# cure-lab/MagicDrive

Measured on AMD Instinct MI355X. Metric: 6-view scenes/sec at 224x400, 50-step DDIM, higher is better.
Workload: dtype bf16; 1 GPU; configs[1]: 6-view 224x400, text-only conditioning (camera_param=None -> CFG off), 50-step DDIM, bf16; scenes_per_gpu=64, ddim_steps=50, scheduler=ddim, parallelism=scene-sharded x1, hipgraph=True, streams=2, output_type=latent

## Files before the change

### include/mdx.h

```cpp
#ifndef MDX_H_
#define MDX_H_

#include <stdint.h>

#ifdef __cplusplus
extern "C" {
#endif

#define MDX_OK 0
#define MDX_EINVAL (-1)
#define MDX_ELAUNCH (-2)
#define MDX_EUNSUPPORTED (-3)

#define MDX_ABI_VERSION 12

#define MDX_EPI_NONE 0
#define MDX_EPI_GEGLU 1
#define MDX_EPI_SILU 2

typedef struct MdxGemmDesc {
    const void* A; const void* W; void* C; const void* R;
    const float* bias; const float* temb; const int32_t* sel_ptr; float* ws;
    int64_t M, N, K;
    int64_t lda, ldw, ldc, ldr;
// ... 32 lines not shown
    const void* X; const void* Wt; void* Y; const void* R;
    const float* bias; const float* temb; const int32_t* sel_ptr; void* reserved_p;
    int64_t B, Hi, Wi, Cin, Ho, Wo, Cout;
    int64_t kh, kw, sh, sw, ph, pw;
    int64_t ldx, ldy, ldr;
    int64_t temb_sel_stride, temb_b_stride;
    int64_t epilogue, x_is_f32, y_is_f32, reserved0;
} MdxConvDirectDesc;
int mdx_conv2d_direct(const MdxConvDirectDesc* d, void* stream);

typedef struct MdxAttnDesc {
    const void* Q; const void* K; const void* Vt; void* O;
    const int32_t* kvmap; const int32_t* tk_dev;
    int64_t B, H, Tq, Tk, d, nsrc;
    int64_t ldq, sQ, ldk, sK, ldv, sV, ldo, sO;
    double scale;
    int64_t joint;
    int64_t q_prescaled;
    int64_t causal;
    int64_t v_rowmajor;
} MdxAttnDesc;
int mdx_attention_bf16(const MdxAttnDesc* d, void* stream);
int mdx_attention_ctx_rows_bf16(const MdxAttnDesc* d, void* stream);

typedef struct MdxGroupNormDesc {
    const void* X; void* Y; const float* gamma; const float* beta;
    int64_t B, HW, C, G, ldx, ldy;
    double eps;
    int64_t silu;
    float* ws; int64_t ws_bytes;
} MdxGroupNormDesc;
int mdx_groupnorm_bf16(const MdxGroupNormDesc* d, void* stream);

typedef struct MdxLayerNormDesc {
    const void* X; void* Y; const float* gamma; const float* beta;
    int64_t M, C, ldx, ldy;
    double eps;
    int64_t reserved0;
} MdxLayerNormDesc;
int mdx_layernorm_bf16(const MdxLayerNormDesc* d, void* stream);

typedef struct MdxSoftmaxDesc {
    const float* X; void* Y;
    int64_t rows, T, ldx, ldy;
    double scale;
    int64_t reserved0;
} MdxSoftmaxDesc;
int mdx_softmax_rows(const MdxSoftmaxDesc* d, void* stream);

#define MDX_EW_ADD 1
#define MDX_EW_COPY 2
#define MDX_EW_UPSAMPLE 3
#define MDX_EW_NCHW_TO_NHWC 4
#define MDX_EW_NHWC_TO_NCHW 5
#define MDX_EW_SILU 6
#define MDX_EW_SCALE 7
typedef struct MdxEwDesc {
    const void* X; void* Y; const int32_t* ymap; const int32_t* xmap;
    int64_t kind, M, C, ldx, ldy;
    int64_t B, Hi, Wi, Ho, Wo;
    int64_t x_is_f32, y_is_f32;
    double alpha;
} MdxEwDesc;
int mdx_elementwise(const MdxEwDesc* d, void* stream);

typedef struct MdxFourierDesc {
// ... 19 lines not shown
    float* x; const float* eps; const float* coef; int32_t* step_ptr; void* x_in; void* reserved_p;
    int64_t n, cfg;
    double guidance;
    int64_t xin_c, xin_ld;
    const float* gv_cond; const float* gv_noise; const uint8_t* gv_mask;
    int64_t gv_mode, gv_view_elems, gv_last_step;
} MdxDdimDesc;
int mdx_cfg_ddim_step(const MdxDdimDesc* d, void* stream);

typedef struct MdxUniPCDesc {
    float* x; const float* eps; const float* coef; int32_t* step_ptr; void* x_in; float* x_last; float* m1; float* m2;
    int64_t n, cfg;
    double guidance;
    int64_t xin_c, xin_ld;
    const float* gv_cond; const float* gv_noise; const uint8_t* gv_mask;
    int64_t gv_mode, gv_view_elems, gv_last_step;
} MdxUniPCDesc;
int mdx_cfg_unipc_step(const MdxUniPCDesc* d, void* stream);

#define MDX_OP_GEMM 1
#define MDX_OP_CONV 2
#define MDX_OP_CONV_DIRECT 3
#define MDX_OP_ATTN 4
#define MDX_OP_GROUPNORM 5
#define MDX_OP_LAYERNORM 6
#define MDX_OP_EW 7
#define MDX_OP_FOURIER 8
#define MDX_OP_GATHER 9
#define MDX_OP_TIMEEMB 10
#define MDX_OP_DDIM 11
#define MDX_OP_UNIPC 12
#define MDX_OP_SOFTMAX 13
#define MDX_OP_ATTN_ROWS 14

#define MDX_DTYPE_BF16 0
#define MDX_DTYPE_F16 1

#define MDX_OP_BYTES 512
typedef struct MdxOp {
    int64_t opcode;
    int64_t dtype;
    unsigned char desc[MDX_OP_BYTES - 16];
} MdxOp;

int mdx_gemm_f16(const MdxGemmDesc* d, void* stream);
int mdx_conv2d_f16(const MdxConvDesc* d, void* stream);
int mdx_conv2d_direct_f16(const MdxConvDirectDesc* d, void* stream);
int mdx_attention_f16(const MdxAttnDesc* d, void* stream);
int mdx_groupnorm_f16(const MdxGroupNormDesc* d, void* stream);
int mdx_layernorm_f16(const MdxLayerNormDesc* d, void* stream);
int mdx_elementwise_f16(const MdxEwDesc* d, void* stream);
int mdx_fourier_embed_f16(const MdxFourierDesc* d, void* stream);
int mdx_gather_rows_f16(const MdxGatherDesc* d, void* stream);
int mdx_timestep_embedding_f16(const MdxTimeEmbDesc* d, void* stream);
int mdx_cfg_ddim_step_f16(const MdxDdimDesc* d, void* stream);
int mdx_cfg_unipc_step_f16(const MdxUniPCDesc* d, void* stream);
int mdx_softmax_rows_f16(const MdxSoftmaxDesc* d, void* stream);
int mdx_attention_ctx_rows_f16(const MdxAttnDesc* d, void* stream);

int mdx_program_run(const MdxOp* ops, int64_t n, void* stream);

int mdx_graph_create(const MdxOp* ops, int64_t n, void** graph_out);
int mdx_graph_launch(void* graph, void* stream);
int mdx_graph_destroy(void* graph);

int mdx_abi_version(void);
const char* mdx_build_id(void);
const char* mdx_last_error(void);
const char* mdx_last_kernel(void);
int mdx_set_option(const char* key, int64_t value);
int mdx_get_option(const char* key, int64_t* value_out);
const char* mdx_option_name(int64_t index);

int mdx_device_info(int64_t* out3);

#ifdef __cplusplus
}
#endif
#endif
```

### magicdrive_amd/_lib.py

```python
from __future__ import annotations

import ctypes as C
import os
from typing import Dict, List, Tuple

_HERE = os.path.dirname(os.path.abspath(__file__))
LIB_PATH = os.environ.get("MDX_LIB_PATH") or os.path.join(_HERE, "libmdx.so")

ABI_VERSION = 12

OP_GEMM, OP_CONV, OP_CONV_DIRECT, OP_ATTN, OP_GROUPNORM, OP_LAYERNORM = 1, 2, 3, 4, 5, 6
OP_EW, OP_FOURIER, OP_GATHER, OP_TIMEEMB, OP_DDIM, OP_UNIPC, OP_SOFTMAX = 7, 8, 9, 10, 11, 12, 13
OP_ATTN_ROWS = 14
OP_BYTES = 512

EPI_NONE, EPI_GEGLU, EPI_SILU = 0, 1, 2
EW_ADD, EW_COPY, EW_UPSAMPLE, EW_NCHW_TO_NHWC, EW_NHWC_TO_NCHW, EW_SILU, EW_SCALE = 1, 2, 3, 4, 5, 6, 7

P, I, D = C.c_void_p, C.c_int64, C.c_double


def _struct(name: str, fields: List[Tuple[str, object]]):
    return type(name, (C.Structure,), {"_fields_": fields})


def _f(kind, names: str):
    return [(n, kind) for n in names.split()]


MdxGemmDesc = _struct("MdxGemmDesc", _f(P, "A W C R bias temb sel_ptr ws") + _f(I, "M N K lda ldw ldc ldr batch sA sW sC sR "
                      "temb_sel_stride temb_b_stride rows_per_b epilogue splitk c_is_f32 ws_bytes") + _f(P, "Vt") + _f(I, "vt_from vt_T vt_ld vt_stride")
                      + _f(D, "ln_eps") + _f(P, "ln_csum ln_scratch") + _f(P, "rowstat_out") + _f(I, "rowstat_parts") + _f(P, "ln_stats") + _f(I, "ln_stats_parts") + _f(P, "Wq"))
MdxConvDesc = _struct("MdxConvDesc", _f(P, "X Wt Y R bias temb sel_ptr ws") + _f(I, "B Hi Wi Cin Ho Wo Cout kh kw sh sw ph pw "
                      "ldx ldy ldr temb_sel_stride temb_b_stride epilogue splitk ws_bytes upsample2x"))
MdxConvDirectDesc = _struct("MdxConvDirectDesc", _f(P, "X Wt Y R bias temb sel_ptr reserved_p") + _f(I, "B Hi Wi Cin Ho Wo Cout kh kw sh sw ph pw "
                            "ldx ldy ldr temb_sel_stride temb_b_stride epilogue x_is_f32 y_is_f32 reserved0"))
MdxAttnDesc = _struct("MdxAttnDesc", _f(P, "Q K Vt O kvmap tk_dev") + _f(I, "B H Tq Tk d nsrc ldq sQ ldk sK ldv sV ldo sO")
                      + _f(D, "scale") + _f(I, "joint q_prescaled causal v_rowmajor"))
MdxGroupNormDesc = _struct("MdxGroupNormDesc", _f(P, "X Y gamma beta") + _f(I, "B HW C G ldx ldy") + _f(D, "eps") + _f(I, "silu") + _f(P, "ws") + _f(I, "ws_bytes"))
MdxLayerNormDesc = _struct("MdxLayerNormDesc", _f(P, "X Y gamma beta") + _f(I, "M C ldx ldy") + _f(D, "eps") + _f(I, "reserved0"))
MdxEwDesc = _struct("MdxEwDesc", _f(P, "X Y ymap xmap") + _f(I, "kind M C ldx ldy B Hi Wi Ho Wo x_is_f32 y_is_f32") + _f(D, "alpha"))
MdxFourierDesc = _struct("MdxFourierDesc", _f(P, "X Y mask null_feat") + _f(I, "n P F ldy"))
MdxGatherDesc = _struct("MdxGatherDesc", _f(P, "T Y idx mask null_row add") + _f(I, "n C ldt ldy n_rows add_period"))
MdxTimeEmbDesc = _struct("MdxTimeEmbDesc", _f(P, "t Y") + _f(I, "n dim flip_sin_to_cos ldy") + _f(D, "freq_shift max_period"))
MdxDdimDesc = _struct("MdxDdimDesc", _f(P, "x eps coef step_ptr x_in reserved_p") + _f(I, "n cfg") + _f(D, "guidance") + _f(I, "xin_c xin_ld")
                      + _f(P, "gv_cond gv_noise gv_mask") + _f(I, "gv_mode gv_view_elems gv_last_step"))
MdxUniPCDesc = _struct("MdxUniPCDesc", _f(P, "x eps coef step_ptr x_in x_last m1 m2") + _f(I, "n cfg") + _f(D, "guidance") + _f(I, "xin_c xin_ld")
                       + _f(P, "gv_cond gv_noise gv_mask") + _f(I, "gv_mode gv_view_elems gv_last_step"))

MdxSoftmaxDesc = _struct("MdxSoftmaxDesc", _f(P, "X Y") + _f(I, "rows T ldx ldy") + _f(D, "scale") + _f(I, "reserved0"))
DESC_OF_OP = {
    OP_GEMM: MdxGemmDesc, OP_CONV: MdxConvDesc, OP_CONV_DIRECT: MdxConvDirectDesc, OP_ATTN: MdxAttnDesc,
    OP_GROUPNORM: MdxGroupNormDesc, OP_LAYERNORM: MdxLayerNormDesc, OP_EW: MdxEwDesc, OP_FOURIER: MdxFourierDesc,
    OP_GATHER: MdxGatherDesc, OP_TIMEEMB: MdxTimeEmbDesc, OP_DDIM: MdxDdimDesc, OP_UNIPC: MdxUniPCDesc, OP_SOFTMAX: MdxSoftmaxDesc,
}
DTYPE_BF16, DTYPE_F16 = 0, 1
ENTRY_OF_OP = {
    OP_GEMM: "mdx_gemm_bf16", OP_CONV: "mdx_conv2d_bf16", OP_CONV_DIRECT: "mdx_conv2d_direct", OP_ATTN: "mdx_attention_bf16",
    OP_GROUPNORM: "mdx_groupnorm_bf16", OP_LAYERNORM: "mdx_layernorm_bf16", OP_EW: "mdx_elementwise",
    OP_FOURIER: "mdx_fourier_embed", OP_GATHER: "mdx_gather_rows", OP_TIMEEMB: "mdx_timestep_embedding", OP_DDIM: "mdx_cfg_ddim_step",
    OP_UNIPC: "mdx_cfg_unipc_step", OP_SOFTMAX: "mdx_softmax_rows",
    OP_ATTN_ROWS: "mdx_attention_ctx_rows_bf16",
}
def entry_name(opcode: int, dtype: int = DTYPE_BF16) -> str:
    n = ENTRY_OF_OP[opcode]
    if dtype == DTYPE_BF16:
        return n
    return (n[:-5] if n.endswith("_bf16") else n) + "_f16"


EXPORTS = sorted(set(ENTRY_OF_OP.values()) | {entry_name(o, DTYPE_F16) for o in ENTRY_OF_OP} | {
    "mdx_program_run", "mdx_graph_create", "mdx_graph_launch", "mdx_graph_destroy",
    "mdx_abi_version", "mdx_build_id", "mdx_last_error", "mdx_last_kernel", "mdx_device_info", "mdx_set_option", "mdx_get_option", "mdx_option_name"})


class MdxOp(C.Structure):
    _fields_ = [("opcode", I), ("dtype", I), ("desc", C.c_ubyte * (OP_BYTES - 16))]


assert C.sizeof(MdxOp) == OP_BYTES
for _d in DESC_OF_OP.values():
    assert C.sizeof(_d) <= OP_BYTES - 16 and C.sizeof(_d) % 8 == 0


class MdxError(RuntimeError):
    pass


_LIB = None


def lib() -> C.CDLL:
    global _LIB
    if _LIB is not None:
        return _LIB
# ... 132 lines not shown
```

### magicdrive_amd/csrc/api.hip

```cpp
#include <cstring>
#include <mutex>
#include <set>
#include <utility>
#include "launch.h"
#include "options.h"
#include <atomic>
#include <cstdlib>

namespace mdx_rt {
char* error_buffer() {
    static thread_local char buf[512] = {0};
    return buf;
}
char* kernel_tag_buffer() {
    static thread_local char buf[128] = {0};
    return buf;
}
int ensure_dyn_smem(const void* kernel, size_t bytes, const char* what) {
    static std::mutex mu;
    static std::set<std::pair<const void*, int>> done;
    int dev = 0;
    hipError_t e = hipGetDevice(&dev);
    if (e != hipSuccess) return mdx::set_error(MDX_ELAUNCH, "hipGetDevice: %s", hipGetErrorString(e));
    std::lock_guard<std::mutex> lk(mu);
// ... 34 lines not shown
    return -1;
}
}
}
namespace mdx_rt {
int64_t opt(int id) { return mdx::g_opt[id].load(std::memory_order_relaxed); }
}

using namespace mdx;

extern "C" int mdx_set_option(const char* key, int64_t value) {
    const int i = find_opt(key);
    if (i < 0) return set_error(MDX_EINVAL, "mdx_set_option: unknown key '%s' (see magicdrive_amd/csrc/options.h)", key ? key : "(null)");
    g_opt[i].store(value, std::memory_order_relaxed);
    return MDX_OK;
}
extern "C" int mdx_get_option(const char* key, int64_t* value_out) {
    const int i = find_opt(key);
    if (i < 0 || !value_out) return set_error(MDX_EINVAL, "mdx_get_option: unknown key '%s'", key ? key : "(null)");
    *value_out = opt(i);
    return MDX_OK;
}
extern "C" const char* mdx_option_name(int64_t index) { return (index >= 0 && index < OPT_COUNT) ? kOptRows[index].key : nullptr; }

static int run_op(const MdxOp* op, hipStream_t st) {
    const void* d = op->desc;
    if (op->dtype == MDX_DTYPE_F16) {
        switch (op->opcode) {
            case MDX_OP_GEMM: return mdx_gemm_f16((const MdxGemmDesc*)d, st);
            case MDX_OP_CONV: return mdx_conv2d_f16((const MdxConvDesc*)d, st);
            case MDX_OP_CONV_DIRECT: return mdx_conv2d_direct_f16((const MdxConvDirectDesc*)d, st);
            case MDX_OP_ATTN: return mdx_attention_f16((const MdxAttnDesc*)d, st);
            case MDX_OP_GROUPNORM: return mdx_groupnorm_f16((const MdxGroupNormDesc*)d, st);
            case MDX_OP_LAYERNORM: return mdx_layernorm_f16((const MdxLayerNormDesc*)d, st);
            case MDX_OP_EW: return mdx_elementwise_f16((const MdxEwDesc*)d, st);
            case MDX_OP_FOURIER: return mdx_fourier_embed_f16((const MdxFourierDesc*)d, st);
            case MDX_OP_GATHER: return mdx_gather_rows_f16((const MdxGatherDesc*)d, st);
            case MDX_OP_TIMEEMB: return mdx_timestep_embedding_f16((const MdxTimeEmbDesc*)d, st);
            case MDX_OP_DDIM: return mdx_cfg_ddim_step_f16((const MdxDdimDesc*)d, st);
            case MDX_OP_UNIPC: return mdx_cfg_unipc_step_f16((const MdxUniPCDesc*)d, st);
            case MDX_OP_SOFTMAX: return mdx_softmax_rows_f16((const MdxSoftmaxDesc*)d, st);
            case MDX_OP_ATTN_ROWS: return mdx_attention_ctx_rows_f16((const MdxAttnDesc*)d, st);
            default: return set_error(MDX_EINVAL, "unknown opcode %ld", (long)op->opcode);
        }
    }
    if (op->dtype != MDX_DTYPE_BF16) return set_error(MDX_EINVAL, "MdxOp.dtype %ld: 0 (bf16) or 1 (fp16)", (long)op->dtype);
    switch (op->opcode) {
        case MDX_OP_GEMM: return mdx_gemm_bf16((const MdxGemmDesc*)d, st);
        case MDX_OP_CONV: return mdx_conv2d_bf16((const MdxConvDesc*)d, st);
        case MDX_OP_CONV_DIRECT: return mdx_conv2d_direct((const MdxConvDirectDesc*)d, st);
        case MDX_OP_ATTN: return mdx_attention_bf16((const MdxAttnDesc*)d, st);
        case MDX_OP_GROUPNORM: return mdx_groupnorm_bf16((const MdxGroupNormDesc*)d, st);
        case MDX_OP_LAYERNORM: return mdx_layernorm_bf16((const MdxLayerNormDesc*)d, st);
        case MDX_OP_EW: return mdx_elementwise((const MdxEwDesc*)d, st);
        case MDX_OP_FOURIER: return mdx_fourier_embed((const MdxFourierDesc*)d, st);
        case MDX_OP_GATHER: return mdx_gather_rows((const MdxGatherDesc*)d, st);
        case MDX_OP_TIMEEMB: return mdx_timestep_embedding((const MdxTimeEmbDesc*)d, st);
        case MDX_OP_DDIM: return mdx_cfg_ddim_step((const MdxDdimDesc*)d, st);
        case MDX_OP_UNIPC: return mdx_cfg_unipc_step((const MdxUniPCDesc*)d, st);
        case MDX_OP_SOFTMAX: return mdx_softmax_rows((const MdxSoftmaxDesc*)d, st);
        case MDX_OP_ATTN_ROWS: return mdx_attention_ctx_rows_bf16((const MdxAttnDesc*)d, st);
        default: return set_error(MDX_EINVAL, "unknown opcode %ld", (long)op->opcode);
    }
}

extern "C" int mdx_program_run(const MdxOp* ops, int64_t n, void* stream) {
    if (!ops && n > 0) return set_error(MDX_EINVAL, "mdx_program_run: null program");
    for (int64_t i = 0; i < n; ++i) {
        int rc = run_op(&ops[i], (hipStream_t)stream);
        if (rc != MDX_OK) {
            char tmp[400];
            strncpy(tmp, error_buffer(), sizeof(tmp) - 1);
            tmp[sizeof(tmp) - 1] = 0;
            return set_error(rc, "op %ld (opcode %ld): %s", (long)i, (long)ops[i].opcode, tmp);
        }
    }
    return MDX_OK;
}

struct GraphHandle {
    hipGraph_t graph;
    hipGraphExec_t exec;
};

extern "C" int mdx_graph_create(const MdxOp* ops, int64_t n, void** graph_out) {
// ... 60 lines not shown
```

### magicdrive_amd/csrc/launch.h

```cpp
#pragma once
#include <hip/hip_runtime.h>
#include <cstdarg>
#include <cstdio>
#include "../../include/mdx.h"

#if defined(MDX_F16) && MDX_F16
#define mdx_gemm_bf16 mdx_gemm_f16
#define mdx_conv2d_bf16 mdx_conv2d_f16
#define mdx_conv2d_direct mdx_conv2d_direct_f16
#define mdx_attention_bf16 mdx_attention_f16
#define mdx_groupnorm_bf16 mdx_groupnorm_f16
#define mdx_layernorm_bf16 mdx_layernorm_f16
#define mdx_elementwise mdx_elementwise_f16
#define mdx_fourier_embed mdx_fourier_embed_f16
#define mdx_gather_rows mdx_gather_rows_f16
#define mdx_timestep_embedding mdx_timestep_embedding_f16
#define mdx_cfg_ddim_step mdx_cfg_ddim_step_f16
#define mdx_cfg_unipc_step mdx_cfg_unipc_step_f16
#define mdx_softmax_rows mdx_softmax_rows_f16
#endif
#ifdef MDX_ATTN_LONG_ENTRY
#undef mdx_attention_bf16
#if defined(MDX_F16) && MDX_F16
#define mdx_attention_bf16 mdx_attention_long_f16
#else
#define mdx_attention_bf16 mdx_attention_long_bf16
#endif
#endif

namespace mdx_rt {
char* error_buffer();
char* kernel_tag_buffer();
int ensure_dyn_smem(const void* kernel, size_t bytes, const char* what);
}

namespace mdx {

using mdx_rt::error_buffer;
using mdx_rt::kernel_tag_buffer;

inline int set_error(int code, const char* fmt, ...) {
    va_list ap;
    va_start(ap, fmt);
    vsnprintf(error_buffer(), 512, fmt, ap);
// ... 29 lines not shown
```

### magicdrive_amd/csrc/norm.hip

```cpp
#include "common.h"
#include "launch.h"
#include "options.h"

namespace mdx {

struct GNParams {
    const bf16_t* X; bf16_t* Y; const float* gamma; const float* beta;
    int B, HW, C, G; long ldx, ldy; float eps; int silu;
};

constexpr int GN_THREADS = 1024;
constexpr int GN_MAX_CPG = 2560;

__device__ __forceinline__ void block_sum2(float& a, float& b, float* red) {
    a = wave_sum(a);
    b = wave_sum(b);
    const int lane = threadIdx.x & 63, wave = threadIdx.x >> 6;
    __syncthreads();
    if (lane == 0) { red[wave] = a; red[16 + wave] = b; }
    __syncthreads();
    float ta = 0.f, tb = 0.f;
#pragma unroll
    for (int i = 0; i < GN_THREADS / 64; ++i) { ta += red[i]; tb += red[16 + i]; }
    a = ta; b = tb;
// ... 511 lines not shown
            for (int e = 0; e < 8; ++e) { const float x = bf2f(f.h[e]); s1 += x; s2 = __builtin_fmaf(x, x, s2); }
        }
    } else {
        for (int c = lane; c < C; c += 64) { const float x = bf2f(xr[c]); s1 += x; s2 = __builtin_fmaf(x, x, s2); }
    }
    s1 = wave_sum(s1); s2 = wave_sum(s2);
    if (lane == 0) {
        *(float2*)(stat + (long)row * 2) = make_float2(s1, s2);
        for (int k = 1; k < parts; ++k) *(float2*)(stat + ((long)k * M + row) * 2) = make_float2(0.f, 0.f);
    }
}
int launch_rowstat(const bf16_t* X, int M, int C, long ldx, float* stat, int parts, hipStream_t st) {
    if (M <= 0) return MDX_OK;
    hipLaunchKernelGGL(rowstat_kernel, dim3((unsigned)((M + 3) / 4)), dim3(256), 0, st, X, M, C, ldx, stat, parts);
    return check_launch("rowstat_kernel");
}
}

extern "C" int mdx_layernorm_bf16(const MdxLayerNormDesc* d, void* stream) {
    if (!d || !d->X || !d->Y || !d->gamma || !d->beta) return set_error(MDX_EINVAL, "mdx_layernorm_bf16: null operand");
    const char* op = "mdx_layernorm_bf16";
    MDX_NEED(need_multiple(op, "C", d->C, 8)); MDX_NEED(need_multiple(op, "ldx", d->ldx, 8)); MDX_NEED(need_multiple(op, "ldy", d->ldy, 8));
    MDX_NEED(need_aligned(op, "X", d->X, 16)); MDX_NEED(need_aligned(op, "Y", d->Y, 16));
    MDX_NEED(need_aligned(op, "gamma", d->gamma, 16)); MDX_NEED(need_aligned(op, "beta", d->beta, 16));
    MDX_NEED(need_int(op, "M", d->M));
    if (d->C <= 0 || d->ldx < d->C || d->ldy < d->C) return set_error(MDX_EINVAL, "%s: need 0 < C <= ldx, ldy", op);
    if (d->C > 8 * 64 * 4) return set_error(MDX_EUNSUPPORTED, "layernorm: C=%ld > 2048", (long)d->C);
    if (d->M <= 0) return MDX_OK;
    LNParams p;
    p.X = (const bf16_t*)d->X; p.Y = (bf16_t*)d->Y; p.gamma = d->gamma; p.beta = d->beta;
    p.M = (int)d->M; p.C = (int)d->C; p.ldx = d->ldx; p.ldy = d->ldy; p.eps = (float)d->eps;
    return launch_layernorm<true>(p, (hipStream_t)stream);
}
```

### magicdrive_amd/csrc/options.h

```cpp
#pragma once
#include <cstdint>

namespace mdx_rt {
int64_t opt(int id);
}

namespace mdx {

#define MDX_OPTIONS(X) \
    X(ATTN_SWZ, 2, "XCD-aware block order of attention.hip: 0 off, 1 per (view, head), 2 per view (all heads of a view on one XCD)") \
    X(ATTN_NW4_BLOCKS, 256L, "attention.hip: 4-wave workgroups from this many blocks") \
    X(ATTN_NW8_BLOCKS, (1L << 40), "attention.hip: 8-wave workgroups from this many blocks") \
    X(ATTN_NW, 0, "force the waves per workgroup of attention.hip (0 = heuristic)") \
    X(ATTN2, 1, "attention2.hip for head dim 40") \
    X(ATTN3, 0, "only in `make ATTN3=1` builds: tools/attn3/attention3.hip (permute-free P, QK of the next kv tile beside this tile's softmax) for the head-dim-40 FOLD launches: self, cross-view, joint") \
    X(ATTN3_WGS, 0, "attention3.hip: persistent workgroups per XCD (0 = automatic: two per CU)") \
    X(ATTN2_PF, 1, "attention2.hip, head dim 40 FOLD 32-query form: permute-free P (PV on 32x32x16 MFMAs, K rows permuted so that a lane's scores are its PV operand)") \
    X(ATTN2_D80, 2, "attention2.hip for head dim 80: 0 never, 1 always, 2 only the two-source cross-view form") \
    X(ATTN2_FOLD, 1, "attention2.hip: subtract the running maximum inside the QK MFMA when Q is pre-scaled (head dim 40)") \
    X(ATTN2_RES, 1, "attention2.hip: kv sequences of <= 3 tiles (text context) resident in LDS, one workgroup per (view, head) walks the query blocks: 0 off, 1 for launches of >= 1024 (view, head) pairs, 2 whenever supported") \
    X(ATTN2_VIEWMAP, 1, "attention2.hip block order: 1 = all heads and query blocks of a view on one XCD (a row's 128-byte lines are shared by the heads), 0 = per (view, head)") \
    X(ATTN2_QT, 0, "32-query tiles per wave in attention2.hip: 0 = automatic (2; 1 for one-source FOLD launches), 1 / 2 = force") \
    X(CONV_OUT_WS, 1, "direct conv with Cout <= 4 and a long K (conv_out): weight-stationary K-parallel kernel (weights in registers, 16 pixels per wave)") \
    X(GEMM_SWZ, 1, "XCD-aware tile order of the generic kernel") \
    X(GEMM_SMALL_TILES, 1, "generic tile choice for small grids (1-4 scenes per call): 64 x 64 for plain GEMMs up to 1408 such tiles and for convs up to 40 k (tile, slab) units, 128 x 128 for larger convs with M < 2048, 128-row GEGLU from M = 512; 0 = the rounds 1-5 rule (128 rows from M = 2048, else 64 x 128)") \
    X(GEMM_BM, 0, "force the generic tile's rows (64 / 128; 0 = heuristic)") \
    X(GEMM_BN, 0, "force the generic tile's columns (64 / 128; 0 = heuristic)") \
    X(GEMM_PIPE, 1, "software-pipelined fragment reads in the generic 128x128x64 tile") \
    X(EPI_WIDE, 1, "16-byte epilogue accesses when alignment allows") \
    X(GEMM_WS, 1, "gemm_ws.hip: 0 off, 1 when M >= 8192, 2 whenever supported") \
    X(GEMM_XL, 1, "gemm_xl.hip: 0 off, 1 cost model, 2 whenever supported") \
    X(XL_K320, 0, "let XL take the K = 320 projections from gemm_ws.hip") \
    X(XL_MIN_TILES, 64, "fewest 256-row tiles an XL launch must have (round 6: 64; 160 until then — 2...8 scenes per call are 2-6 % faster with the lower bound, 12+ scenes and 1 scene do not care: profiles/r06_lat1_small_grids.log)") \
    X(XL_BN, 0, "force an XL tile width (160 / 256 / 320; 0 = cost model)") \
    X(XL_GEGLU320, 0, "K = 320 GEGLU on the 256-wide XL tile instead of gemm_ws.hip") \
    X(GEMM_BM256, 0, "generic 256x128 8-wave tile from M >= value (0 = never)") \
    X(GEMM_TIMING, 0, "s_memtime stamps of the generic kernel into the op workspace") \
    X(GEMM_BK, 64, "generic tile slab depth (64 or 32)") \
    X(GEMM_FLATTEN, 1, "batched shared-A GEMM as ONE col_split XL launch") \
    X(CONV_CIMAJOR, 1, "channel-block-major K order of implicit-GEMM convs") \
    X(WS_SLOTS, 512, "workgroup slots the gemm_ws M walkers are sized for") \
    X(XL_TIMING, 0, "per-workgroup s_memtime stamps into the op workspace") \
    X(GN_REVERSE, 1, "two-stage GroupNorm: statistics pass reads the tensor back to front (Infinity-Cache reuse between producer / passes)") \
    X(GN_FINALIZE_CHUNKS, 16, "two-stage GroupNorm: with more chunks per image than this the chunk partials are combined once by gn_finalize_kernel (0 = always in the apply pass)") \
    X(GN_ONE_KERNEL_ELEMS, (4L << 20), "GroupNorm tensors of at most this many elements (all images) take the one-launch kernel (one workgroup per (image, group)) instead of the two streaming passes") \
    X(GN_TWO_STAGE, 1, "streaming two-stage GroupNorm for maps >= 32768 elements") \
    X(XL_PERSIST, 1, "256x256 XL GEMMs (plain / GEGLU, optional residual) on the persistent kernel gemm_xlp_kernel") \
    X(XD, 0, "W-direct persistent GEMM (gemm_xd.hip: weights global -> registers, finished tile stored under the next tile's main loop) for the 256x256 XL GEMMs whose descriptor carries Wq (K % 128 == 0, K >= 640); bit-identical to gemm_xlp_kernel, measured 0.89-1.04x of it (profiles/r06_xd_ab.log): off by default") \
    X(XL_RASTER, 2, "XL tile order: 0 row-major, 1 XCD-strided M-tiles, 2 XCD-blocked (M-group x N-group panels per XCD)") \
    X(XL_GM, 0, "XL_RASTER 2: force the M-tiles per panel (0 = cost model, xl_layout.h: raster_shape)") \
    X(XL_GN, 0, "XL_RASTER 2: force the N-tiles per panel (0 = cost model)") \
    X(STREAMS, 2, "host side (pipeline): HIP streams a pipe() call spreads its scene chunks over (chunks of >= 16 scenes, one plan + hipGraph each)") \
    X(PLAN_CACHE, 6, "host side (pipeline): sampler plans (captured graphs + buffers) kept per pipeline (LRU); a multi-stream call pins one plan per chunk") \
    X(CHECK_TIMESTEPS, 0, "host side (schedulers): 1 = a device-resident timestep that is not in the scheduler's list raises (one sync per step) instead of poisoning the sample with NaN") \
    X(LN_FUSE, 1, "MdxGemmDesc.ln_eps: 1 = gemm_ws.hip normalises the rows in-kernel, 0 = always normalise into ln_scratch first (A/B)") \
    X(LN_STATS, 1, "MdxGemmDesc.rowstat_out / ln_stats: 1 = row statistics travel from the producer's store phase to the fused LayerNorm, 0 = round-5 behaviour (nothing emitted, in-kernel sums, GEGLU through ln_scratch) (A/B)")

enum Opt : int {
#define MDX_OPT_ENUM(key, dflt, doc) OPT_##key,
    MDX_OPTIONS(MDX_OPT_ENUM)
#undef MDX_OPT_ENUM
    OPT_COUNT
};

using mdx_rt::opt;

}
```

### magicdrive_amd/engine.py

```python
from __future__ import annotations

from typing import Dict, List, Optional, Sequence, Tuple

import torch

from . import _lib as L
from . import ops as O
from . import packing as PK
from .networks.spec import heads_at

BF16, F32 = torch.bfloat16, torch.float32


def q_prescale(head_dim: int) -> float:
    return float(head_dim) ** -0.5 * 1.4426950408889634


class PackedNet:

    def __init__(self, sd: Dict[str, torch.Tensor], device, dtype=BF16):
        assert dtype in (torch.bfloat16, torch.float16), "the kernels take bf16 or fp16 operands (fp32 accumulate)"
        self.sd = sd
        self.device = device
        self.dtype = dtype
        self.cache: Dict[Tuple, torch.Tensor] = {}

    def has(self, key: str) -> bool:
        return key in self.sd

    def _get(self, tag, keys, fn):
        ck = (tag,) + tuple(keys)
        if ck not in self.cache:
            self.cache[ck] = fn(*[self.sd[k].detach().float() for k in keys]).to(self.device)
        return self.cache[ck]

    def lin(self, key, scale: float = 1.0):
        return self._get(("lin", scale), [key], lambda w: (w.reshape(w.shape[0], -1) * scale).contiguous().to(self.dtype))

    def conv(self, key):
# ... 170 lines not shown
class ActSlice:

    __slots__ = ("parent", "c0", "B", "H", "W", "C")

    def __init__(self, parent: Act, c0: int, c1: int):
        self.parent, self.c0, self.B, self.H, self.W, self.C = parent, c0, parent.B, parent.H, parent.W, c1 - c0

    @property
    def tok(self):
        return self.parent.tok[:, self.c0:self.c0 + self.C]

    @property
    def bhwc(self):
        return self.parent.bhwc[..., self.c0:self.c0 + self.C]

    @property
    def btc(self):
        return self.parent.btc[..., self.c0:self.c0 + self.C]


def upsample_conv_folds(device, fold, Hi: int, Wi: int, Ho: int, Wo: int, cin: int, B: int = 0, ldx: int = 0) -> bool:
    if fold is None:
        fold = torch.device(device).type == "cuda"
    if not (bool(fold) and cin % 64 == 0 and Hi * Wi + 256 < (1 << 24) and PK.upsample_fold_ok(Hi, Ho) and PK.upsample_fold_ok(Wi, Wo)):
        return False
    if B and (Ho != 2 * Hi or Wo != 2 * Wi) and (B * Hi * Wi + Wi + 2) * (ldx or cin) * 2 >= 0x7fff0000:
        return False
    return True


class Builder:

    fold_upsample = None

    def __init__(self, cfg, device, n_views: int, n_cam: int, ws_mb: int = 64, dtype=BF16):
        self.cfg = cfg
        self.device = device
        self.B = n_views
        self.n_cam = n_cam
        self.dtype = dtype
        self.pool = Pool(device, dtype)
        self.ops: List[object] = []
        self.ctx_tk_dev: Optional[torch.Tensor] = None
        self.ctx_tk_per_view = False
        self.ws = torch.empty(ws_mb * 1024 * 1024 // 4, dtype=F32, device=device)
        self.groups = cfg["norm_num_groups"]
        self.eps = cfg["norm_eps"]
        pair = cfg["neighboring_view_pair"]
        pair = {int(k): [int(x) for x in v] for k, v in pair.items()}
        self.nattn = cfg.get("neighboring_attn_type", "add")
        if self.nattn not in ("add", "concat", "self"):
            raise NotImplementedError(f"Unknown type: {self.nattn}")
        counts = [len(pair[c]) for c in range(n_cam)]
        self.xv_counts: Optional[List[int]] = None
        self.xv_bo_scale = 1.0
        if self.nattn == "add":
            for c, n in enumerate(counts):
                if n > 2:
                    raise NotImplementedError(f"neighboring_attn_type 'add': view {c} lists {n} neighbours; the summed cross-view form handles at most 2 per view")
            if max(counts) == 0:
                raise RuntimeError("neighboring_view_pair lists no neighbour for any view: there is no cross-view attention to run (torch.cat(): expected a non-empty list of Tensors)")
            self.xv_nsrc = 1 if all(n == 1 for n in counts) else 2
            if len(set(counts)) == 1:
                self.xv_bo_scale = float(counts[0])
            else:
                self.xv_counts = [counts[i % n_cam] for i in range(n_views)]
        elif self.nattn == "concat":
            if len(set(counts)) != 1 or counts[0] == 0:
                raise RuntimeError(f"neighboring_attn_type 'concat' needs the same, non-zero number of neighbours for every view (got {counts}): "
                                   "the reference's torch.cat of the per-view kv sequences fails too (blocks.py:125-132)")
            self.xv_nsrc = counts[0]
        else:
            self.xv_nsrc = n_cam
        assert self.xv_nsrc <= 8, "joint cross-view attention handles <= 8 sources"
        kv = []
        for i in range(n_views):
            base = (i // n_cam) * n_cam
            srcs = list(range(n_cam)) if self.nattn == "self" else pair[i % n_cam]
            kv += [base + nb for nb in srcs] + [-1] * (self.xv_nsrc - len(srcs))
        self.kvmap = torch.tensor(kv, dtype=torch.int32, device=device)
        self.kvmap._mdx_present = sum(1 for x in kv if x >= 0)

    def emit(self, op):
        self.ops.append(op)
        return op

    def new(self, B, H, W, C) -> Act:
        return Act(self.pool.get((B * H * W, C)), B, H, W, C)

    def free(self, a):
        if isinstance(a, ActSlice):
            return
        self.pool.put(a.t if isinstance(a, Act) else a)

    def groupnorm(self, net, pre, x: Act, eps, silu, name) -> Act:
        y = self.new(x.B, x.H, x.W, x.C)
        self.emit(O.GroupNorm(x.btc, y.btc, net.vec(pre + "weight"), net.vec(pre + "bias"), self.groups, eps, silu, ws=self.ws, name=name))
        return y

    def layernorm(self, net, pre, x: torch.Tensor, name) -> torch.Tensor:
        y = self.pool.get(tuple(x.shape))
        self.emit(O.LayerNorm(x, y, net.vec(pre + "weight"), net.vec(pre + "bias"), 1e-5, name=name))
        return y

    @staticmethod
    def wq_of(W: torch.Tensor, M: int, epilogue: int) -> Optional[torch.Tensor]:
        if W.dim() != 2 or not W.is_contiguous() or epilogue not in (L.EPI_NONE, L.EPI_GEGLU) or not L.get_option("XD"):
            return None
        N, K = W.shape
        if K % 128 or K < 640 or N % 16 or ((M + 255) // 256) * ((N + 255) // 256) < 512:
            return None
        wq = getattr(W, "_mdx_wq", None)
        if wq is None:
            wq = PK.pack_wq(W)
            W._mdx_wq = wq
        return wq

    def gemm(self, A, W, N_out, bias=None, R=None, epilogue=L.EPI_NONE, name="", out=None, **kw) -> torch.Tensor:
        C = out if out is not None else self.pool.get((A.shape[0], N_out))
        if "Wq" not in kw and not any(kw.get(k) is not None for k in ("Vt", "temb", "rowstat")) and not kw.get("ln_eps"):
            kw["Wq"] = self.wq_of(W, A.shape[0], epilogue)
        self.emit(O.Gemm(A, W, C, bias=bias, R=R, epilogue=epilogue, ws=self.ws, name=name, **kw))
        return C

    def resnet(self, net, pre, x: Act, temb: "TembTable", name, out=None) -> Act:
        cout = net.sd[pre + "conv1.weight"].shape[0]
        a = self.groupnorm(net, pre + "norm1.", x, self.eps, True, name + ".norm1")
        h = self.new(x.B, x.H, x.W, cout)
        off = temb.offset[pre + "time_emb_proj.weight"]
        self.emit(O.Conv(a.bhwc, net.conv(pre + "conv1.weight"), h.bhwc, bias=net.vec(pre + "conv1.bias"),
# ... 317 lines not shown
```

### magicdrive_amd/ops.py

```python
from __future__ import annotations

from dataclasses import dataclass, field
from typing import Optional

import torch

from . import _lib as L

BF16 = torch.bfloat16
F16 = torch.float16
H16 = (BF16, F16)
F32 = torch.float32


def _p(t: Optional[torch.Tensor]):
    return None if t is None else t.data_ptr()


def _chk(cond: bool, msg: str):
    if not cond:
        raise ValueError(msg)


def _rows2d(t: torch.Tensor):
# ... 269 lines not shown
            opcode = L.OP_ATTN_ROWS
        _chk(self.nsrc >= 1 and (self.nsrc <= 8 if self.joint else self.nsrc <= 2), f"attn {self.name}: nsrc={self.nsrc} (joint={self.joint})")
        return opcode, d


@dataclass
class GroupNorm:
    X: torch.Tensor
    Y: torch.Tensor
    gamma: torch.Tensor
    beta: torch.Tensor
    groups: int
    eps: float
    silu: bool = False
    ws: Optional[torch.Tensor] = None
    name: str = ""
    opcode = L.OP_GROUPNORM

    def lower(self):
        B, HW, Cc = self.X.shape
        _chk(self.X.stride(2) == 1 and self.Y.stride(2) == 1 and self.Y.shape == self.X.shape, f"gn {self.name}: layout")
        _chk(B == 1 or (self.X.stride(0) == HW * self.X.stride(1) and self.Y.stride(0) == HW * self.Y.stride(1)), f"gn {self.name}: batch stride")
        _chk(self.gamma.dtype == F32 and self.beta.dtype == F32 and self.gamma.numel() == Cc, f"gn {self.name}: affine")
        d = L.MdxGroupNormDesc()
        d.X, d.Y, d.gamma, d.beta = _p(self.X), _p(self.Y), _p(self.gamma), _p(self.beta)
        d.B, d.HW, d.C, d.G, d.ldx, d.ldy = B, HW, Cc, self.groups, self.X.stride(1), self.Y.stride(1)
        d.eps, d.silu = float(self.eps), int(self.silu)
        if self.ws is not None:
            d.ws = _p(self.ws); d.ws_bytes = self.ws.numel() * self.ws.element_size()
        return self.opcode, d


@dataclass
class LayerNorm:
    X: torch.Tensor
    Y: torch.Tensor
    gamma: torch.Tensor
    beta: torch.Tensor
    eps: float = 1e-5
    name: str = ""
    opcode = L.OP_LAYERNORM

    def lower(self):
        M, Cc, ldx = _rows2d(self.X)
        M2, C2, ldy = _rows2d(self.Y)
        _chk(M == M2 and Cc == C2, f"ln {self.name}: shapes")
        d = L.MdxLayerNormDesc()
        d.X, d.Y, d.gamma, d.beta = _p(self.X), _p(self.Y), _p(self.gamma), _p(self.beta)
        d.M, d.C, d.ldx, d.ldy, d.eps = M, Cc, ldx, ldy, float(self.eps)
        return self.opcode, d


@dataclass
class Softmax:
    X: torch.Tensor
    Y: torch.Tensor
    T: int
    scale: float = 1.0
    name: str = ""
    opcode = L.OP_SOFTMAX

    def lower(self):
        _chk(self.X.dtype == F32 and self.Y.dtype in H16 and self.X.dim() == 2 and self.Y.dim() == 2, "softmax: dtypes / rank")
        _chk(self.X.stride(1) == 1 and self.Y.stride(1) == 1 and self.X.shape[0] == self.Y.shape[0], "softmax: layout")
        _chk(0 < self.T <= self.X.shape[1] and self.T <= self.Y.shape[1], "softmax: T")
        d = L.MdxSoftmaxDesc()
# ... 269 lines not shown
```

Measured before the change: 7.390 scenes/s.

## Add register-resident single-read GroupNorm kernel for large activation maps

Adds a new GroupNorm kernel that loads each workgroup's slab of k groups into registers once, computes the mean and variance from those registers with two block reductions, then applies scale, shift and optional SiLU before writing. The builder routes GroupNorms larger than the one-kernel threshold to this op when the shape fits, replacing the streaming two-pass path that reads the input twice. Images are mapped across XCDs by block index. The cost is very high register pressure with 1024-thread blocks and possibly low occupancy, and shapes the plan cannot serve fall back to the old kernels.

```diff
diff --git a/include/mdx.h b/include/mdx.h
--- a/include/mdx.h
+++ b/include/mdx.h
@@ -88,6 +88,8 @@
 } MdxGroupNormDesc;
 int mdx_groupnorm_bf16(const MdxGroupNormDesc* d, void* stream);
 
+int mdx_groupnorm_resident_bf16(const MdxGroupNormDesc* d, void* stream);
+
 typedef struct MdxLayerNormDesc {
     const void* X; void* Y; const float* gamma; const float* beta;
     int64_t M, C, ldx, ldy;
@@ -173,6 +175,7 @@
 #define MDX_OP_UNIPC 12
 #define MDX_OP_SOFTMAX 13
 #define MDX_OP_ATTN_ROWS 14
+#define MDX_OP_GROUPNORM_RESIDENT 15
 
 #define MDX_DTYPE_BF16 0
 #define MDX_DTYPE_F16 1
@@ -189,6 +192,7 @@
 int mdx_conv2d_direct_f16(const MdxConvDirectDesc* d, void* stream);
 int mdx_attention_f16(const MdxAttnDesc* d, void* stream);
 int mdx_groupnorm_f16(const MdxGroupNormDesc* d, void* stream);
+int mdx_groupnorm_resident_f16(const MdxGroupNormDesc* d, void* stream);
 int mdx_layernorm_f16(const MdxLayerNormDesc* d, void* stream);
 int mdx_elementwise_f16(const MdxEwDesc* d, void* stream);
 int mdx_fourier_embed_f16(const MdxFourierDesc* d, void* stream);
diff --git a/magicdrive_amd/_lib.py b/magicdrive_amd/_lib.py
--- a/magicdrive_amd/_lib.py
+++ b/magicdrive_amd/_lib.py
@@ -12,6 +12,7 @@
 OP_GEMM, OP_CONV, OP_CONV_DIRECT, OP_ATTN, OP_GROUPNORM, OP_LAYERNORM = 1, 2, 3, 4, 5, 6
 OP_EW, OP_FOURIER, OP_GATHER, OP_TIMEEMB, OP_DDIM, OP_UNIPC, OP_SOFTMAX = 7, 8, 9, 10, 11, 12, 13
 OP_ATTN_ROWS = 14
+OP_GROUPNORM_RESIDENT = 15
 OP_BYTES = 512
 
 EPI_NONE, EPI_GEGLU, EPI_SILU = 0, 1, 2
@@ -61,6 +62,7 @@
     OP_FOURIER: "mdx_fourier_embed", OP_GATHER: "mdx_gather_rows", OP_TIMEEMB: "mdx_timestep_embedding", OP_DDIM: "mdx_cfg_ddim_step",
     OP_UNIPC: "mdx_cfg_unipc_step", OP_SOFTMAX: "mdx_softmax_rows",
     OP_ATTN_ROWS: "mdx_attention_ctx_rows_bf16",
+    OP_GROUPNORM_RESIDENT: "mdx_groupnorm_resident_bf16",
 }
 def entry_name(opcode: int, dtype: int = DTYPE_BF16) -> str:
     n = ENTRY_OF_OP[opcode]
diff --git a/magicdrive_amd/csrc/api.hip b/magicdrive_amd/csrc/api.hip
--- a/magicdrive_amd/csrc/api.hip
+++ b/magicdrive_amd/csrc/api.hip
@@ -90,6 +90,7 @@
             case MDX_OP_CONV_DIRECT: return mdx_conv2d_direct_f16((const MdxConvDirectDesc*)d, st);
             case MDX_OP_ATTN: return mdx_attention_f16((const MdxAttnDesc*)d, st);
             case MDX_OP_GROUPNORM: return mdx_groupnorm_f16((const MdxGroupNormDesc*)d, st);
+            case MDX_OP_GROUPNORM_RESIDENT: return mdx_groupnorm_resident_f16((const MdxGroupNormDesc*)d, st);
             case MDX_OP_LAYERNORM: return mdx_layernorm_f16((const MdxLayerNormDesc*)d, st);
             case MDX_OP_EW: return mdx_elementwise_f16((const MdxEwDesc*)d, st);
             case MDX_OP_FOURIER: return mdx_fourier_embed_f16((const MdxFourierDesc*)d, st);
@@ -109,6 +110,7 @@
         case MDX_OP_CONV_DIRECT: return mdx_conv2d_direct((const MdxConvDirectDesc*)d, st);
         case MDX_OP_ATTN: return mdx_attention_bf16((const MdxAttnDesc*)d, st);
         case MDX_OP_GROUPNORM: return mdx_groupnorm_bf16((const MdxGroupNormDesc*)d, st);
+        case MDX_OP_GROUPNORM_RESIDENT: return mdx_groupnorm_resident_bf16((const MdxGroupNormDesc*)d, st);
         case MDX_OP_LAYERNORM: return mdx_layernorm_bf16((const MdxLayerNormDesc*)d, st);
         case MDX_OP_EW: return mdx_elementwise((const MdxEwDesc*)d, st);
         case MDX_OP_FOURIER: return mdx_fourier_embed((const MdxFourierDesc*)d, st);
diff --git a/magicdrive_amd/csrc/gn_route.h b/magicdrive_amd/csrc/gn_route.h
--- /dev/null
+++ b/magicdrive_amd/csrc/gn_route.h
@@ -0,0 +1,43 @@
+#pragma once
+
+#if defined(__HIPCC__) || defined(__HIP__)
+#define MDX_GN_ROUTE_HD __host__ __device__ __forceinline__
+#else
+#define MDX_GN_ROUTE_HD inline
+#endif
+
+namespace mdx_route {
+
+constexpr int GNR_THREADS = 1024;
+constexpr int GNR_MAX_NV = 22;
+constexpr int GNR_MAX_CH = 1024;
+constexpr int GNR_MAX_K = 32;
+constexpr int GNR_PAIR_NV = 4;
+constexpr long GNR_ONE_KERNEL_ELEMS = 4L << 20;
+
+MDX_GN_ROUTE_HD int gn_resident_nv(long HW, long C, long G, long k) {
+    if (HW <= 0 || C <= 0 || G <= 0 || C % G || k <= 0 || k > GNR_MAX_K || G % k) return 0;
+    const long cpg = C / G, ch = k * cpg;
+    if (cpg < 8 || cpg % 2 || ch % 8 || ch > GNR_MAX_CH) return 0;
+    const long vpr = ch / 8, rpp = GNR_THREADS / vpr;
+    const long nv = (HW + rpp - 1) / rpp;
+    return nv <= GNR_MAX_NV ? (int)nv : 0;
+}
+
+MDX_GN_ROUTE_HD int gn_resident_plan(long B, long HW, long C, long G, long ldx, long ldy, long alignment, long min_elems = GNR_ONE_KERNEL_ELEMS) {
+    if (B <= 0 || HW <= 0 || C <= 0 || G <= 0 || C % G) return 0;
+    if (ldx < C || ldy < C || ldx % 8 || ldy % 8 || alignment < 16) return 0;
+    const long ldm = ldx > ldy ? ldx : ldy;
+    if (HW * ldm >= (1L << 31) || B > 0x7fffffffL / G) return 0;
+    if (B * HW * C <= min_elems) return 0;
+    const long kmax = G < GNR_MAX_K ? G : GNR_MAX_K;
+    for (long k = kmax; k >= 1; --k) {
+        const int nv = gn_resident_nv(HW, C, G, k);
+        if (nv && nv <= GNR_PAIR_NV) return (int)k;
+    }
+    for (long k = kmax; k >= 1; --k)
+        if (gn_resident_nv(HW, C, G, k)) return (int)k;
+    return 0;
+}
+
+}
diff --git a/magicdrive_amd/csrc/launch.h b/magicdrive_amd/csrc/launch.h
--- a/magicdrive_amd/csrc/launch.h
+++ b/magicdrive_amd/csrc/launch.h
@@ -10,6 +10,7 @@
 #define mdx_conv2d_direct mdx_conv2d_direct_f16
 #define mdx_attention_bf16 mdx_attention_f16
 #define mdx_groupnorm_bf16 mdx_groupnorm_f16
+#define mdx_groupnorm_resident_bf16 mdx_groupnorm_resident_f16
 #define mdx_layernorm_bf16 mdx_layernorm_f16
 #define mdx_elementwise mdx_elementwise_f16
 #define mdx_fourier_embed mdx_fourier_embed_f16
diff --git a/magicdrive_amd/csrc/norm.hip b/magicdrive_amd/csrc/norm.hip
--- a/magicdrive_amd/csrc/norm.hip
+++ b/magicdrive_amd/csrc/norm.hip
@@ -567,3 +567,197 @@
     p.M = (int)d->M; p.C = (int)d->C; p.ldx = d->ldx; p.ldy = d->ldy; p.eps = (float)d->eps;
     return launch_layernorm<true>(p, (hipStream_t)stream);
 }
+
+#include "gn_route.h"
+
+namespace mdx {
+
+struct GNRParams {
+    const bf16_t* X; bf16_t* Y; const float* gamma; const float* beta;
+    int B, HW, C, G, k, cpg, vpr, rpp; long ldx, ldy; float eps; int silu;
+};
+
+using mdx_route::GNR_THREADS;
+using mdx_route::GNR_MAX_CH;
+using mdx_route::GNR_MAX_K;
+
+__device__ __forceinline__ float gnr_silu(float x) { return x * __builtin_amdgcn_rcpf(1.0f + __expf(-x)); }
+
+template <int NV>
+__global__ __launch_bounds__(GNR_THREADS) void gn_resident_kernel(GNRParams p) {
+    __shared__ float part[2][GNR_THREADS];
+    __shared__ float gst[2][GNR_MAX_K];
+    __shared__ __attribute__((aligned(16))) float lsc[GNR_MAX_CH], lsh[GNR_MAX_CH];
+    const int tid = threadIdx.x, lane = tid & 63, wave = tid >> 6;
+    const int nb = p.G / p.k;
+    const int xcd = blockIdx.x & 7, kq = blockIdx.x >> 3;
+    const int sib = kq % nb, b = (kq / nb) * 8 + xcd;
+    if (b >= p.B) return;
+    const int cpg = p.cpg, vpr = p.vpr, rpp = p.rpp, HW = p.HW, kc = p.k * cpg;
+    const int ch0 = sib * kc;
+    int rl = tid / vpr, col = tid - rl * vpr;
+    const bool live = rl < rpp;
+    if (!live) { rl = 0; col = 0; }
+    const int glo = (col * 8) / cpg;
+    const int split = min(8, (glo + 1) * cpg - col * 8);
+    const int ldx = (int)p.ldx, ldy = (int)p.ldy;
+    const bf16_t* xb = p.X + (long)b * HW * p.ldx + ch0 + col * 8;
+    bf16_t* yb = p.Y + (long)b * HW * p.ldy + ch0 + col * 8;
+
+    constexpr int UM = NV - 4;
+    const int cg = tid < kc ? tid : 0;
+    const float gam = p.gamma[ch0 + cg], bet = p.beta[ch0 + cg];
+    uint4 d[NV];
+#pragma unroll
+    for (int u = 0; u < NV; ++u) {
+        const int px = rl + u * rpp;
+        d[u] = *(const uint4*)(xb + (u < UM || px < HW ? px : HW - 1) * ldx);
+    }
+    auto keep_packed = [&]() {
+#pragma unroll
+        for (int u = 0; u < NV; ++u) asm volatile("" : "+v"(d[u].x), "+v"(d[u].y), "+v"(d[u].z), "+v"(d[u].w));
+    };
+    keep_packed();
+    float okf[4];
+#pragma unroll
+    for (int i = 0; i < 4; ++i) {
+        const int u = UM + i;
+        const bool ok = rl + u * rpp < HW;
+        okf[i] = ok ? 1.f : 0.f;
+        d[u].x = ok ? d[u].x : 0u; d[u].y = ok ? d[u].y : 0u; d[u].z = ok ? d[u].z : 0u; d[u].w = ok ? d[u].w : 0u;
+    }
+    if (tid < kc) { lsc[tid] = gam; lsh[tid] = bet; }
+
+    const float inv_n = 1.0f / ((float)HW * (float)cpg);
+    auto reduce = [&](const float* s, int which) {
+        float lo = 0.f, hi = 0.f;
+#pragma unroll
+        for (int e = 0; e < 8; ++e) { if (e < split) lo += s[e]; else hi += s[e]; }
+        part[0][tid] = lo; part[1][tid] = hi;
+        __syncthreads();
+        for (int g = wave; g < p.k; g += GNR_THREADS / 64) {
+            const int c0 = (g * cpg) / 8, c1 = ((g + 1) * cpg - 1) / 8;
+            float acc = 0.f;
+            for (int r = lane; r < rpp; r += 64)
+                for (int c = c0; c <= c1; ++c) acc += part[(c * 8) / cpg == g ? 0 : 1][r * vpr + c];
+            acc = wave_sum(acc);
+            if (lane == 0) gst[which][g] = acc;
+        }
+        __syncthreads();
+    };
+
+    float s[8];
+#pragma unroll
+    for (int e = 0; e < 8; ++e) s[e] = 0.f;
+    __builtin_amdgcn_sched_barrier(0);
+#pragma unroll
+    for (int u = 0; u < NV; ++u) {
+        Frag8 f; f.u = d[u];
+#pragma unroll
+        for (int e = 0; e < 8; ++e) s[e] += bf2f(f.h[e]);
+        __builtin_amdgcn_sched_barrier(0);
+    }
+    reduce(s, 0);
+    keep_packed();
+    const int ghi = glo + 1 < p.k ? glo + 1 : glo;
+    const float mlo = gst[0][glo] * inv_n, mhi = gst[0][ghi] * inv_n;
+    float mp[4];
+#pragma unroll
+    for (int q = 0; q < 4; ++q) { mp[q] = 2 * q < split ? mlo : mhi; asm volatile("" : "+v"(mp[q])); }
+#pragma unroll
+    for (int e = 0; e < 8; ++e) s[e] = 0.f;
+    __builtin_amdgcn_sched_barrier(0);
+#pragma unroll
+    for (int u = 0; u < NV; ++u) {
+        Frag8 f; f.u = d[u];
+#pragma unroll
+        for (int e = 0; e < 8; ++e) {
+            float dl = bf2f(f.h[e]) - mp[e >> 1];
+            if (u >= UM) dl *= okf[u - UM < 0 ? 0 : u - UM];
+            s[e] = __builtin_fmaf(dl, dl, s[e]);
+        }
+        __builtin_amdgcn_sched_barrier(0);
+    }
+    reduce(s, 1);
+    keep_packed();
+    if (tid < kc) {
+        const int g = tid / cpg;
+        const float sc = rsqrtf(gst[1][g] * inv_n + p.eps) * lsc[tid];
+        lsc[tid] = sc; lsh[tid] = lsh[tid] - gst[0][g] * inv_n * sc;
+    }
+    __syncthreads();
+    if (!live) return;
+    int rls = rl;
+    asm volatile("" : "+v"(rls));
+    constexpr bool LEAN = NV > 16;
+    float4 a[2], h[2];
+    if constexpr (!LEAN) {
+        a[0] = *(const float4*)(lsc + col * 8); a[1] = *(const float4*)(lsc + col * 8 + 4);
+        h[0] = *(const float4*)(lsh + col * 8); h[1] = *(const float4*)(lsh + col * 8 + 4);
+    }
+    __builtin_amdgcn_sched_barrier(0);
+#pragma unroll
+    for (int u = 0; u < NV; ++u) {
+        const int px = rls + u * rpp;
+        Frag8 f; f.u = d[u];
+        uint32_t w[4];
+#pragma unroll
+        for (int q = 0; q < 2; ++q) {
+            float4 sc, sh;
+            if constexpr (LEAN) {
+                asm volatile("" ::: "memory");
+                sc = *(const float4*)(lsc + col * 8 + q * 4); sh = *(const float4*)(lsh + col * 8 + q * 4);
+            } else {
+                sc = a[q]; sh = h[q];
+            }
+            float y0 = __builtin_fmaf(bf2f(f.h[q * 4 + 0]), sc.x, sh.x), y1 = __builtin_fmaf(bf2f(f.h[q * 4 + 1]), sc.y, sh.y);
+            float y2 = __builtin_fmaf(bf2f(f.h[q * 4 + 2]), sc.z, sh.z), y3 = __builtin_fmaf(bf2f(f.h[q * 4 + 3]), sc.w, sh.w);
+            if (p.silu) { y0 = gnr_silu(y0); y1 = gnr_silu(y1); y2 = gnr_silu(y2); y3 = gnr_silu(y3); }
+            w[q * 2] = pack2bf(y0, y1); w[q * 2 + 1] = pack2bf(y2, y3);
+        }
+        if (u < UM || px < HW) *(uint4*)(yb + px * ldy) = make_uint4(w[0], w[1], w[2], w[3]);
+        __builtin_amdgcn_sched_barrier(0);
+    }
+}
+
+static int gn_resident_check(const char* op, const MdxGroupNormDesc* d) {
+    if (!d || !d->X || !d->Y || !d->gamma || !d->beta) return set_error(MDX_EINVAL, "%s: null operand", op);
+    if (d->G <= 0 || d->C % d->G) return set_error(MDX_EINVAL, "groupnorm: C=%ld not divisible by G=%ld", (long)d->C, (long)d->G);
+    MDX_NEED(need_int(op, "B", d->B)); MDX_NEED(need_int(op, "HW", d->HW)); MDX_NEED(need_int(op, "C", d->C)); MDX_NEED(need_int(op, "G", d->G));
+    MDX_NEED(need_aligned(op, "gamma", d->gamma, 16)); MDX_NEED(need_aligned(op, "beta", d->beta, 16)); MDX_NEED(need_aligned(op, "ws", d->ws, 16));
+    MDX_NEED(need_aligned(op, "X", d->X, 2)); MDX_NEED(need_aligned(op, "Y", d->Y, 2));
+    if (d->C <= 0 || d->ldx < d->C || d->ldy < d->C) return set_error(MDX_EINVAL, "%s: need 0 < C <= ldx, ldy", op);
+    return MDX_OK;
+}
+
+}
+
+extern "C" int mdx_groupnorm_resident_bf16(const MdxGroupNormDesc* d, void* stream) {
+    const char* op = "mdx_groupnorm_resident_bf16";
+    if (int rc = gn_resident_check(op, d)) return rc;
+    if (d->B <= 0 || d->HW <= 0) return MDX_OK;
+    const long mode = opt(OPT_GN_RESIDENT);
+    if (mode <= 0) return set_error(MDX_EUNSUPPORTED, "%s: switched off (option GN_RESIDENT = 0)", op);
+    const long align = (((uintptr_t)d->X | (uintptr_t)d->Y) & 15) == 0 ? 16 : 1;
+    int k = mdx_route::gn_resident_plan(d->B, d->HW, d->C, d->G, d->ldx, d->ldy, align, mode >= 2 ? 0 : opt(OPT_GN_ONE_KERNEL_ELEMS));
+    const long force_k = opt(OPT_GN_RESIDENT_K);
+    if (k && force_k > 0) k = mdx_route::gn_resident_nv(d->HW, d->C, d->G, force_k) ? (int)force_k : 0;
+    if (!k)
+        return set_error(MDX_EUNSUPPORTED, "%s: [%ld][%ld][%ld] G=%ld ldx=%ld ldy=%ld is not served (gn_route.h: slab, 16-byte rows, size rule)", op,
+                         (long)d->B, (long)d->HW, (long)d->C, (long)d->G, (long)d->ldx, (long)d->ldy);
+    GNRParams p;
+    p.X = (const bf16_t*)d->X; p.Y = (bf16_t*)d->Y; p.gamma = d->gamma; p.beta = d->beta;
+    p.B = (int)d->B; p.HW = (int)d->HW; p.C = (int)d->C; p.G = (int)d->G; p.ldx = d->ldx; p.ldy = d->ldy;
+    p.eps = (float)d->eps; p.silu = (int)d->silu;
+    p.k = k; p.cpg = p.C / p.G; p.vpr = k * p.cpg / 8; p.rpp = GNR_THREADS / p.vpr;
+    const int nv = mdx_route::gn_resident_nv(p.HW, p.C, p.G, k);
+    const dim3 grid((unsigned)(((p.B + 7) / 8) * 8 * (p.G / k))), block(GNR_THREADS);
+    hipStream_t st = (hipStream_t)stream;
+    if (nv <= 4) hipLaunchKernelGGL(gn_resident_kernel<4>, grid, block, 0, st, p);
+    else if (nv <= 8) hipLaunchKernelGGL(gn_resident_kernel<8>, grid, block, 0, st, p);
+    else if (nv <= 12) hipLaunchKernelGGL(gn_resident_kernel<12>, grid, block, 0, st, p);
+    else if (nv <= 16) hipLaunchKernelGGL(gn_resident_kernel<16>, grid, block, 0, st, p);
+    else if (nv <= 20) hipLaunchKernelGGL(gn_resident_kernel<20>, grid, block, 0, st, p);
+    else hipLaunchKernelGGL(gn_resident_kernel<mdx_route::GNR_MAX_NV>, grid, block, 0, st, p);
+    return check_launch("gn_resident_kernel");
+}
diff --git a/magicdrive_amd/csrc/options.h b/magicdrive_amd/csrc/options.h
--- a/magicdrive_amd/csrc/options.h
+++ b/magicdrive_amd/csrc/options.h
@@ -45,6 +45,8 @@
     X(GN_FINALIZE_CHUNKS, 16, "two-stage GroupNorm: with more chunks per image than this the chunk partials are combined once by gn_finalize_kernel (0 = always in the apply pass)") \
     X(GN_ONE_KERNEL_ELEMS, (4L << 20), "GroupNorm tensors of at most this many elements (all images) take the one-launch kernel (one workgroup per (image, group)) instead of the two streaming passes") \
     X(GN_TWO_STAGE, 1, "streaming two-stage GroupNorm for maps >= 32768 elements") \
+    X(GN_RESIDENT, 1, "register-resident one-read GroupNorm (gn_resident_kernel, an op of its own: MDX_OP_GROUPNORM_RESIDENT): 0 off (the engine emits none, the entry point refuses), 1 where gn_route.h says so (tensors above GN_ONE_KERNEL_ELEMS), 2 whenever the kernel can serve the shape") \
+    X(GN_RESIDENT_K, 0, "force the groups per workgroup of gn_resident_kernel (0 = gn_route.h: the widest block that fits; tools/gn_bench.py sweeps it)") \
     X(XL_PERSIST, 1, "256x256 XL GEMMs (plain / GEGLU, optional residual) on the persistent kernel gemm_xlp_kernel") \
     X(XD, 0, "W-direct persistent GEMM (gemm_xd.hip: weights global -> registers, finished tile stored under the next tile's main loop) for the 256x256 XL GEMMs whose descriptor carries Wq (K % 128 == 0, K >= 640); bit-identical to gemm_xlp_kernel, measured 0.89-1.04x of it (profiles/r06_xd_ab.log): off by default") \
     X(XL_RASTER, 2, "XL tile order: 0 row-major, 1 XCD-strided M-tiles, 2 XCD-blocked (M-group x N-group panels per XCD)") \
diff --git a/magicdrive_amd/engine.py b/magicdrive_amd/engine.py
--- a/magicdrive_amd/engine.py
+++ b/magicdrive_amd/engine.py
@@ -5,6 +5,7 @@
 import torch
 
 from . import _lib as L
+from . import gn_route as GR
 from . import ops as O
 from . import packing as PK
 from .networks.spec import heads_at
@@ -241,6 +242,8 @@
 class Builder:
 
     fold_upsample = None
+
+    gn_resident = None
 
     def __init__(self, cfg, device, n_views: int, n_cam: int, ws_mb: int = 64, dtype=BF16):
         self.cfg = cfg
@@ -304,7 +307,17 @@
 
     def groupnorm(self, net, pre, x: Act, eps, silu, name) -> Act:
         y = self.new(x.B, x.H, x.W, x.C)
-        self.emit(O.GroupNorm(x.btc, y.btc, net.vec(pre + "weight"), net.vec(pre + "bias"), self.groups, eps, silu, ws=self.ws, name=name))
+        xv, yv = x.btc, y.btc
+        kind = O.GroupNorm
+        mode, floor = self.gn_resident, GR.GNR_ONE_KERNEL_ELEMS
+        if mode is None:
+            mode = L.get_option("GN_RESIDENT") if torch.device(self.device).type == "cuda" else 0
+            floor = L.get_option("GN_ONE_KERNEL_ELEMS") if mode > 0 else floor
+        if mode > 0:
+            align = 16 if (xv.data_ptr() | yv.data_ptr()) % 16 == 0 else 1
+            if GR.gn_resident_plan(x.B, x.H * x.W, x.C, self.groups, xv.stride(1), yv.stride(1), align, 0 if mode >= 2 else floor):
+                kind = O.GroupNormResident
+        self.emit(kind(xv, yv, net.vec(pre + "weight"), net.vec(pre + "bias"), self.groups, eps, silu, ws=self.ws, name=name))
         return y
 
     def layernorm(self, net, pre, x: torch.Tensor, name) -> torch.Tensor:
diff --git a/magicdrive_amd/gn_route.py b/magicdrive_amd/gn_route.py
--- /dev/null
+++ b/magicdrive_amd/gn_route.py
@@ -0,0 +1,40 @@
+from __future__ import annotations
+
+GNR_THREADS = 1024
+GNR_MAX_NV = 22
+GNR_MAX_CH = 1024
+GNR_MAX_K = 32
+GNR_PAIR_NV = 4
+GNR_ONE_KERNEL_ELEMS = 4 << 20
+
+
+def gn_resident_nv(HW: int, C: int, G: int, k: int) -> int:
+    if HW <= 0 or C <= 0 or G <= 0 or C % G or k <= 0 or k > GNR_MAX_K or G % k:
+        return 0
+    cpg = C // G
+    ch = k * cpg
+    if cpg < 8 or cpg % 2 or ch % 8 or ch > GNR_MAX_CH:
+        return 0
+    vpr = ch // 8
+    rpp = GNR_THREADS // vpr
+    nv = (HW + rpp - 1) // rpp
+    return nv if nv <= GNR_MAX_NV else 0
+
+
+def gn_resident_plan(B: int, HW: int, C: int, G: int, ldx: int, ldy: int, alignment: int, min_elems: int = GNR_ONE_KERNEL_ELEMS) -> int:
+    if B <= 0 or HW <= 0 or C <= 0 or G <= 0 or C % G:
+        return 0
+    if ldx < C or ldy < C or ldx % 8 or ldy % 8 or alignment < 16:
+        return 0
+    if HW * max(ldx, ldy) >= (1 << 31) or B > 0x7fffffff // G:
+        return 0
+    if B * HW * C <= min_elems:
+        return 0
+    ks = range(min(G, GNR_MAX_K), 0, -1)
+    for k in ks:
+        if 0 < gn_resident_nv(HW, C, G, k) <= GNR_PAIR_NV:
+            return k
+    for k in ks:
+        if gn_resident_nv(HW, C, G, k):
+            return k
+    return 0
diff --git a/magicdrive_amd/ops.py b/magicdrive_amd/ops.py
--- a/magicdrive_amd/ops.py
+++ b/magicdrive_amd/ops.py
@@ -325,6 +325,11 @@
 
 
 @dataclass
+class GroupNormResident(GroupNorm):
+    opcode = L.OP_GROUPNORM_RESIDENT
+
+
+@dataclass
 class LayerNorm:
     X: torch.Tensor
     Y: torch.Tensor
```

New measurement: 7.496 scenes/s (median of 6 runs). +1.4%, better.
